# Connor-Guo/torcheval

Hardware: AMD Instinct MI355X
Metric: metric-updates/sec (whole node) MulticlassAccuracy bs=8192 at 1/2/4/8 MI355X (higher is better)
Workload: dtype fp32; 1 GPU; model=MulticlassAccuracy, global_batch=8192, num_classes=1000, batch_per_gpu=8192, average=micro, parallelism=dp1

## Files before the change

### csrc/bindings/counts.cpp

```cpp
#include <ATen/ATen.h>
#include <torch/csrc/utils/pybind.h>
#include <torch/library.h>

#include "tea_kernels.h"
#include "tea_torch.h"

namespace {

using namespace tea_torch;

void cls_counts(const Tensor& input, const Tensor& target, int64_t k, int64_t num_classes,
                const optional<Tensor>& micro_correct, const optional<Tensor>& micro_total,
                const optional<Tensor>& cls_correct, const optional<Tensor>& cls_label,
                const optional<Tensor>& cls_pred, const optional<Tensor>& confusion,
                const optional<Tensor>& err, int64_t max_blocks,
                const optional<Tensor>& micro_incorrect, const optional<Tensor>& micro_total2,
                const optional<Tensor>& cls_fp) {
  check_gpu(input, "input");
  check_gpu(target, "target");
  TORCH_CHECK(target.dim() == 1, "cls_counts: target must be 1-D");
  TORCH_CHECK(input.dim() == 1 || input.dim() == 2, "cls_counts: input must be 1-D or 2-D");
  TORCH_CHECK(input.size(0) == target.size(0), "cls_counts: first dims differ");
  TORCH_CHECK(target.is_contiguous(), "cls_counts: target must be contiguous");
  DeviceGuard guard(input.device());
  tea::ClsCountsArgs a;
  Tensor in = input;
  if (input.dim() == 2) {
    if (in.stride(1) != 1) in = in.contiguous();
    a.c = in.size(1);
    a.row_stride = in.stride(0);
    TORCH_CHECK(a.c < (int64_t(1) << 31), "cls_counts: too many classes");
    TORCH_CHECK(k >= 1 && k <= a.c || a.c == 0, "cls_counts: k out of range");
    if (num_classes <= 0) num_classes = a.c;
    TORCH_CHECK(num_classes == a.c, "cls_counts: num_classes must match input.size(1)");
  } else {
    if (!in.is_contiguous()) in = in.contiguous();
    TORCH_CHECK(k == 1, "cls_counts: k > 1 needs 2-D scores");
  }
  const int64_t C = num_classes;
  a.input = in.data_ptr();
  a.in_dt = dt_of(in);
  a.n = in.size(0);
  a.target = target.data_ptr();
  a.tg_dt = dt_of(target);
  a.k = static_cast<int>(k);
  a.num_classes = C;
  a.micro_correct = f32_out(micro_correct, input, 1, "micro_correct");
  a.micro_total = f32_out(micro_total, input, 1, "micro_total");
  a.cls_correct = f32_out(cls_correct, input, C, "cls_correct");
  a.cls_label = f32_out(cls_label, input, C, "cls_label");
  a.cls_pred = f32_out(cls_pred, input, C, "cls_pred");
  a.confusion = f32_out(confusion, input, C * C, "confusion");
  a.micro_incorrect = f32_out(micro_incorrect, input, 1, "micro_incorrect");
  a.micro_total2 = f32_out(micro_total2, input, 1, "micro_total2");
  a.cls_fp = f32_out(cls_fp, input, C, "cls_fp");
  TORCH_CHECK(!(k > 1 && (a.cls_pred || a.confusion || a.cls_fp)),
              "cls_counts: predictions are undefined for k > 1");
  TORCH_CHECK((a.cls_correct || a.cls_label || a.cls_pred || a.confusion || a.cls_fp) == false ||
                  C > 0,
              "cls_counts: num_classes required for histograms");
  if ((a.err = err_ptr(err, input, "cls_counts")) != nullptr) {
    if (err->numel() >= 3) a.err_max = a.err + 1;
    a.check_target = 1;
  }
  a.max_blocks = static_cast<int>(max_blocks);
  const hipStream_t stream = stream_for(input);
  if (a.micro_correct || a.micro_incorrect) a.fold_ws = fold_workspace(input, stream);
  const int rc = tea::launch_cls_counts(a, stream);
  TORCH_CHECK(rc != -1, "cls_counts: unsupported input dtype ", input.scalar_type());
  check_launch(rc, "cls_counts");
}

bool micro_accuracy_update(const Tensor& input, const Tensor& target, const Tensor& correct,
                           const Tensor& total, int64_t num_classes, const optional<Tensor>& pend) {
  if (!input.is_cuda() || input.dim() != 2 || target.dim() != 1) return false;
  const int64_t n = input.size(0), c = input.size(1);
  if (target.size(0) != n || c <= 0 || c >= (int64_t(1) << 31) || input.stride(1) != 1) return false;
  if (num_classes > 0 && c != num_classes) return false;
  const auto st = input.scalar_type();
  if (st != at::kFloat && st != at::kBFloat16 && st != at::kHalf) return false;
  switch (target.scalar_type()) {
    case at::kLong: case at::kInt: case at::kShort: case at::kChar: case at::kByte: case at::kBool:
      break;
    default: return false;
  }
  if (!target.is_contiguous()) return false;
  const auto dev = input.device();
  if (target.device() != dev || correct.device() != dev || total.device() != dev) return false;
  if (correct.scalar_type() != at::kFloat || total.scalar_type() != at::kFloat ||
      correct.numel() != 1 || total.numel() != 1)
    return false;
  DeviceGuard guard(dev);
  tea::ClsCountsArgs a;
  a.input = input.data_ptr();
  a.in_dt = dt_of(input);
  a.n = n;
  a.c = c;
  a.row_stride = input.stride(0);
  a.target = target.data_ptr();
  a.tg_dt = dt_of(target);
  a.k = 1;
  a.num_classes = c;
  a.micro_correct = correct.data_ptr<float>();
  a.micro_total = total.data_ptr<float>();
  const hipStream_t stream = stream_for(input);
  if (pend.has_value()) {
    if (pend->scalar_type() != at::kLong || pend->numel() < tea::kPendCells * tea::kPendStride ||
        pend->device() != dev || !pend->is_contiguous())
      return false;
    a.pend = reinterpret_cast<unsigned long long*>(pend->data_ptr<int64_t>());
  } else {
    a.fold_ws = fold_workspace(input, stream);
  }
  check_launch(tea::launch_cls_counts(a, stream), "micro_accuracy_update");
  return true;
}

void micro_accuracy_finish(const Tensor& pend, const Tensor& correct, const Tensor& total,
                           const optional<Tensor>& out) {
  check_gpu(pend, "pend");
  TORCH_CHECK(pend.scalar_type() == at::kLong && pend.is_contiguous() &&
                  pend.numel() >= tea::kPendCells * tea::kPendStride,
              "micro_accuracy_finish: pend must be int64 [>= 512]");
  TORCH_CHECK(correct.scalar_type() == at::kFloat && total.scalar_type() == at::kFloat && correct.numel() == 1 &&
                  total.numel() == 1 && correct.device() == pend.device() && total.device() == pend.device(),
              "micro_accuracy_finish: float32 scalar states on the pending cells' device");
  float* o = nullptr;
  if (out.has_value()) {
    TORCH_CHECK(out->scalar_type() == at::kFloat && out->numel() == 1 && out->device() == pend.device(),
                "micro_accuracy_finish: out must be a float32 scalar");
    o = out->data_ptr<float>();
  }
  DeviceGuard guard(pend.device());
  check_launch(tea::launch_micro_finish(reinterpret_cast<unsigned long long*>(pend.data_ptr<int64_t>()),
                                        correct.data_ptr<float>(), total.data_ptr<float>(), o, stream_for(pend)),
               "micro_accuracy_finish");
}

Tensor rank_scores(const Tensor& input, const Tensor& target, int64_t mode, int64_t k,
                   const optional<Tensor>& err) {
  check_gpu(input, "input");
  check_gpu(target, "target");
  TORCH_CHECK(input.dim() == 2 && target.dim() == 1 && input.size(0) == target.size(0),
              "rank_scores: input [n, c] and target [n] expected");
  TORCH_CHECK(mode == 0 || mode == 1, "rank_scores: mode must be 0 (hit) or 1 (reciprocal)");
  TORCH_CHECK(input.size(1) < (int64_t(1) << 31), "rank_scores: too many columns");
  DeviceGuard guard(input.device());
  Tensor in = input.stride(1) == 1 ? input : input.contiguous();
  Tensor tg = target.contiguous();
  tea::RankArgs a;
  a.input = in.data_ptr();
  a.in_dt = dt_of(in);
  a.n = in.size(0);
  a.c = in.size(1);
  a.row_stride = in.stride(0);
  a.target = tg.data_ptr();
  a.tg_dt = dt_of(tg);
  a.mode = static_cast<int>(mode);
  a.k = static_cast<int>(k);
  Tensor out = at::empty({a.n}, input.options().dtype(at::kFloat));
  a.out = out.data_ptr<float>();
  a.err = err_ptr(err, input, "rank_scores");
  const int rc = tea::launch_rank_scores(a, stream_for(input));
  TORCH_CHECK(rc != -1, "rank_scores: unsupported input dtype ", input.scalar_type());
  check_launch(rc, "rank_scores");
  return out;
}

void binary_counts(const Tensor& input, const Tensor& target, const optional<Tensor>& weight,
                   double threshold, const optional<Tensor>& tp, const optional<Tensor>& fp,
                   const optional<Tensor>& tn, const optional<Tensor>& fn,
                   const optional<Tensor>& total, int64_t strict, int64_t max_blocks,
                   const optional<Tensor>& tp2, const optional<Tensor>& fp2,
                   const optional<Tensor>& tn2, const optional<Tensor>& fn2) {
  check_gpu(input, "input");
  check_gpu(target, "target");
  TORCH_CHECK(input.numel() == target.numel(), "binary_counts: size mismatch");
  DeviceGuard guard(input.device());
  Tensor in = input.contiguous();
  Tensor tg = target.contiguous();
  Tensor w;
  tea::BinaryCountsArgs a;
  if (weight.has_value()) {
    w = weight->contiguous();
    TORCH_CHECK(w.numel() == in.numel(), "binary_counts: weight size mismatch");
    a.weight = w.data_ptr();
    a.w_dt = dt_of(w);
  }
  a.input = in.data_ptr();
  a.in_dt = dt_of(in);
  a.target = tg.data_ptr();
  a.tg_dt = dt_of(tg);
  a.n = in.numel();
  a.threshold = threshold_as(in, threshold);
  a.threshold64 = threshold;
  a.strict_binary = static_cast<int>(strict);
  a.out[0] = f32_out(tp, input, 1, "tp");
  a.out[1] = f32_out(fp, input, 1, "fp");
  a.out[2] = f32_out(tn, input, 1, "tn");
  a.out[3] = f32_out(fn, input, 1, "fn");
  a.total = f32_out(total, input, 1, "total");
  a.out2[0] = f32_out(tp2, input, 1, "tp2");
  a.out2[1] = f32_out(fp2, input, 1, "fp2");
  a.out2[2] = f32_out(tn2, input, 1, "tn2");
  a.out2[3] = f32_out(fn2, input, 1, "fn2");
  a.max_blocks = static_cast<int>(max_blocks);
  check_launch(tea::launch_binary_counts(a, stream_for(input)), "binary_counts");
}

void multilabel_counts(const Tensor& input, const Tensor& target, double threshold, int64_t k,
                       int64_t criteria, const Tensor& num_correct, const optional<Tensor>& num_total,
                       double total) {
  check_gpu(input, "input");
  check_gpu(target, "target");
  TORCH_CHECK(input.dim() == 2 && target.sizes() == input.sizes(),
              "multilabel_counts: input/target must be [n, c] of equal shape");
  TORCH_CHECK(input.stride(1) == 1 && target.stride(1) == 1,
              "multilabel_counts: rows must be contiguous");
  TORCH_CHECK(num_correct.scalar_type() == at::kFloat && num_correct.numel() == 1 &&
                  num_correct.device() == input.device(),
              "multilabel_counts: num_correct must be a float32 scalar on the input device");
  TORCH_CHECK(criteria >= 0 && criteria <= 4, "multilabel_counts: bad criteria");
  TORCH_CHECK(k == 0 || (k >= 1 && k <= input.size(1) && input.size(1) <= tea::multilabel_max_topk_cols()),
              "multilabel_counts: top-k needs 1 <= k <= c <= ", tea::multilabel_max_topk_cols());
  TORCH_CHECK(criteria != 1 || input.numel() < (int64_t{1} << 31),
              "multilabel_counts: hamming counts must fit 31 bits per launch");
  DeviceGuard guard(input.device());
  hipStream_t stream = stream_for(input);
  tea::MultilabelArgs a;
  a.x = input.data_ptr();
  a.x_dt = dt_of(input);
  a.x_row_stride = input.stride(0);
  a.t = target.data_ptr();
  a.t_dt = dt_of(target);
  a.t_row_stride = target.stride(0);
  a.n = input.size(0);
  a.c = input.size(1);
  a.threshold = threshold_as(input, threshold);
  a.k = static_cast<int>(k);
  a.criteria = static_cast<int>(criteria);
  a.num_correct = num_correct.data_ptr<float>();
  if (num_total.has_value()) {
    TORCH_CHECK(num_total->scalar_type() == at::kFloat && num_total->numel() == 1,
                "multilabel_counts: num_total must be a float32 scalar");
    a.num_total = num_total->data_ptr<float>();
    a.total = total;
  }
  a.fold_ws = fold_workspace(input, stream);
  const int rc = tea::launch_multilabel(a, stream);
  TORCH_CHECK(rc != -1, "multilabel_counts: unsupported dtypes ", input.scalar_type(), "/",
              target.scalar_type());
  check_launch(rc, "multilabel_counts");
}

void binned_counts(const Tensor& input, const Tensor& target, const Tensor& thr, int64_t mode,
                   const optional<Tensor>& tp, const optional<Tensor>& fp,
                   const optional<Tensor>& fn, int64_t uniform) {
  check_gpu(input, "input");
  TORCH_CHECK(input.dim() == 2, "binned_counts: input must be a 2-D view [n, c]");
  TORCH_CHECK(thr.dim() == 1 && thr.scalar_type() == at::kFloat && thr.is_contiguous(),
              "binned_counts: thresholds must be a contiguous float32 vector");
  DeviceGuard guard(input.device());
  tea::BinnedArgs a;
  a.input = input.data_ptr();
  a.in_dt = dt_of(input);
  a.n = input.size(0);
// ... 217 lines not shown
```

### csrc/include/tea_kernels.h

```cpp
#pragma once

#include <hip/hip_runtime_api.h>
#include <stdint.h>

#include "tea_types.h"

namespace tea {

struct ClsCountsArgs {
  const void* input = nullptr;
  DType in_dt = DType::f32;
  int64_t n = 0;
  int64_t c = 0;
  int64_t row_stride = 0;
  const void* target = nullptr;
  DType tg_dt = DType::i64;
  int k = 1;
  int64_t num_classes = 0;
  float* micro_correct = nullptr;
  float* micro_incorrect = nullptr;
  float* micro_total = nullptr;
  float* micro_total2 = nullptr;
  float* cls_correct = nullptr;
  float* cls_label = nullptr;
  float* cls_pred = nullptr;
  float* cls_fp = nullptr;
  float* confusion = nullptr;
  int* err = nullptr;
  int* err_max = nullptr;
  int check_target = 0;
  unsigned long long* fold_ws = nullptr;
  unsigned long long* pend = nullptr;
  int max_blocks = 0;
};
int launch_cls_counts(const ClsCountsArgs& a, hipStream_t stream);
constexpr int kPendCells = 64;
constexpr int kPendStride = 8;
int launch_micro_finish(unsigned long long* pend, float* correct, const float* total, float* out, hipStream_t stream);

struct BinaryCountsArgs {
  const void* input = nullptr;
  DType in_dt = DType::f32;
  const void* target = nullptr;
  DType tg_dt = DType::f32;
  const void* weight = nullptr;
  DType w_dt = DType::f32;
  int64_t n = 0;
  float threshold = 0.5f;
  double threshold64 = 0.5;
  int strict_binary = 0;
  float* out[4] = {nullptr, nullptr, nullptr, nullptr};
  float* out2[4] = {nullptr, nullptr, nullptr, nullptr};
  float* total = nullptr;
  int max_blocks = 0;
};
int launch_binary_counts(const BinaryCountsArgs& a, hipStream_t stream);

struct RankArgs {
  const void* input = nullptr;
  DType in_dt = DType::f32;
  int64_t n = 0;
  int64_t c = 0;
  int64_t row_stride = 0;
  const void* target = nullptr;
  DType tg_dt = DType::i64;
  int mode = 0;
  int k = 0;
  float* out = nullptr;
  int* err = nullptr;
};
int launch_rank_scores(const RankArgs& a, hipStream_t stream);

}

namespace tea {

struct AucScanArgs {
  int payload_kind = 0;
  const void* sorted = nullptr;
  DType key_dt = DType::f32;
  int64_t key_stride = 0;
  const int64_t* order = nullptr;
  const int32_t* order32 = nullptr;
  int64_t order_stride = 0;
  const void* target = nullptr;
  DType tg_dt = DType::f32;
  int64_t target_stride = 0;
  const void* weight = nullptr;
  DType w_dt = DType::f32;
  int64_t weight_stride = 0;
  int class_mode = 0;
  int64_t rows = 0;
  int64_t n = 0;
  double* out_auroc = nullptr;
  double* out_auprc = nullptr;
  const uint32_t* sort_fault = nullptr;
  const double* init = nullptr;
  double* out_raw = nullptr;
  void* ab = nullptr;
  void* tsum = nullptr;
  void* tstart = nullptr;
  void* tarea = nullptr;
  void* totals = nullptr;
  int32_t* tcnt = nullptr;
  int32_t* cstart = nullptr;
  int64_t* sizes = nullptr;
  const int64_t* row_off = nullptr;
  float* out_prec = nullptr;
  float* out_rec = nullptr;
  void* out_thr = nullptr;
  float min_precision = 0.f;
  float* s_rec = nullptr;
  void* s_thr = nullptr;
  int32_t* gstar = nullptr;
  int32_t* glo = nullptr;
  float* out_max_recall = nullptr;
  void* out_best_thr = nullptr;
};
int64_t auc_scan_workspace_bytes(int64_t rows, int64_t n);
int launch_auc_scan(AucScanArgs a, void* workspace, hipStream_t stream);
int64_t curve_workspace_bytes(int64_t rows, int64_t n, bool rafp);
constexpr int kMergeTile = 2048;
int64_t merge_splits_count(int64_t n);
int launch_merge_desc(const float* ka, const uint32_t* va, int64_t na, uint32_t base_a, const float* kb,
                      const uint32_t* vb, int64_t nb, uint32_t base_b, float* ko, uint32_t* vo, int64_t* splits,
                      hipStream_t stream);
int launch_curve_count(AucScanArgs& a, void* workspace, bool rafp, hipStream_t stream);
int launch_curve_emit(AucScanArgs a, void* workspace, bool rafp, hipStream_t stream);
int launch_rafp(AucScanArgs a, void* workspace, hipStream_t stream);

}

namespace tea {

struct BinnedArgs {
  const void* input = nullptr;
  DType in_dt = DType::f32;
  int64_t n = 0;
  int64_t c = 0;
  int64_t in_row_stride = 0;
  int64_t in_col_stride = 0;
  const void* target = nullptr;
  DType tg_dt = DType::i64;
  int mode = 0;
  int64_t tg_row_stride = 0;
  int64_t tg_col_stride = 0;
  const float* thr = nullptr;
  int T = 0;
  int uniform = 0;
  unsigned* ws = nullptr;
  unsigned* slab = nullptr;
  float* tp = nullptr;
  float* fp = nullptr;
  float* fn = nullptr;
  int64_t out_k_stride = 0;
  int64_t out_c_stride = 0;
};
int64_t binned_workspace_words(int T, int64_t c);
int64_t binned_slab_words(int T, int64_t c);
struct BinnedFinalizeArgs {
  const float* tp = nullptr;
  const float* fp = nullptr;
  const float* fn = nullptr;
  int64_t k_stride = 0, r_stride = 0;
  int T = 0;
  int64_t rows = 0;
  double* out_auroc = nullptr;
  float* out_auprc = nullptr;
  float* out_prec = nullptr;
  float* out_rec = nullptr;
};
int launch_binned_finalize(const BinnedFinalizeArgs& a, hipStream_t stream);
int launch_binned(const BinnedArgs& a, hipStream_t stream);

}

namespace tea {

struct MomentsArgs {
  const void* x = nullptr;
  DType x_dt = DType::f32;
  int64_t x_row_stride = 0, x_col_stride = 0;
  const void* t = nullptr;
  DType t_dt = DType::f32;
  int64_t t_row_stride = 0, t_col_stride = 0;
  const void* w = nullptr;
  DType w_dt = DType::f32;
  int64_t w_stride = 0;
// ... 715 lines not shown
```

### csrc/kernels/classification.hip

```cpp
#include <algorithm>
#include <cstdlib>

#include "tea_common.h"
#include "tea_fold.h"
#include "tea_kernels.h"
#include "tea_rowload.h"

namespace tea {

namespace {

constexpr int kBlock = 256;
constexpr int kWavesPerBlock = kBlock / kWave;
constexpr int kChunkLoads = 4;
constexpr int kNarrowMaxC = 32;

template <int KIND, int VEC>
__device__ __forceinline__ void load_vec(const void* row, int col, float (&v)[VEC]) {
  if constexpr (KIND == 0 && VEC == 4) {
    const float4 x = *reinterpret_cast<const float4*>(static_cast<const float*>(row) + col);
    v[0] = x.x;
    v[1] = x.y;
    v[2] = x.z;
    v[3] = x.w;
// ... 271 lines not shown
        if (base + CHUNK < C) load_chunk<KIND, VEC, UNAL>(rp, base + CHUNK, C, lane, nx);
        finish_chunk<VEC, UNAL>(v, base, C, lane);
#pragma unroll
        for (int u = 0; u < kChunkLoads; ++u)
#pragma unroll
          for (int e = 0; e < VEC; ++e) cnt += v[u][e] > xt;
      }
      cnt = wave_sum(cnt);
      correct = t_ok && cnt < a.k;
    }
    if (lane == 0) {
      correct_acc += correct;
      rows_acc += 1;
      row_hist(h, a.num_classes, t, pred, correct, a.err, a.check_target, a.err_max);
    }
  }
  block_micro(a, correct_acc, rows_acc);
}


template <int CTRL>
__device__ __forceinline__ float dpp_f32(float x) {
  return __int_as_float(__builtin_amdgcn_update_dpp(0, __float_as_int(x), CTRL, 0xf, 0xf, false));
}

__device__ __forceinline__ float wave_max_dpp(float x) {
  x = fmaximum(x, dpp_f32<0xB1>(x));
  x = fmaximum(x, dpp_f32<0x4E>(x));
  x = fmaximum(x, dpp_f32<0x141>(x));
  x = fmaximum(x, dpp_f32<0x140>(x));
  const float r0 = __int_as_float(__builtin_amdgcn_readlane(__float_as_int(x), 0));
  const float r1 = __int_as_float(__builtin_amdgcn_readlane(__float_as_int(x), 16));
  const float r2 = __int_as_float(__builtin_amdgcn_readlane(__float_as_int(x), 32));
  const float r3 = __int_as_float(__builtin_amdgcn_readlane(__float_as_int(x), 48));
  return fmaximum(fmaximum(r0, r1), fmaximum(r2, r3));
}

template <int NV>
struct RowVals;
template <>
struct RowVals<16> {
  typedef float type __attribute__((ext_vector_type(16)));
};
template <>
struct RowVals<32> {
  typedef float type __attribute__((ext_vector_type(32)));
};

template <int KIND, typename TGT, bool UNAL = false>
__device__ __forceinline__ void micro_rows(const void* __restrict__ input, const TGT* __restrict__ target, int64_t n,
                                           int C, int64_t row_stride, uint32_t& correct_acc, uint32_t& rows_acc) {
  constexpr int VEC = KIND == 0 ? 4 : 8;
  constexpr int NV = kChunkLoads * VEC;
  constexpr int STEP = kWave * VEC;
  typedef typename RowVals<NV>::type vec_t;
  const int lane = lane_id();
  const int64_t nwaves = static_cast<int64_t>(gridDim.x) * kWavesPerBlock;
  for (int64_t row = static_cast<int64_t>(blockIdx.x) * kWavesPerBlock + wave_id(); row < n; row += nwaves) {
    const char* rp = static_cast<const char*>(input) + row * row_stride * kind_bytes<KIND>;
    float f[kChunkLoads][VEC];
#pragma unroll
    for (int u = 0; u < kChunkLoads; ++u) load_row_vec<KIND, VEC, UNAL>(rp, u * STEP + lane * VEC, C, f[u]);
    const int64_t t = target[row];
    if constexpr (UNAL) unal_fix_tail<kChunkLoads>(f, 0, C, lane);
    vec_t v;
#pragma unroll
    for (int u = 0; u < kChunkLoads; ++u)
#pragma unroll
      for (int e = 0; e < VEC; ++e) v[u * VEC + e] = f[u][e];
    float m = fmaximum(v[0], v[1]);
#pragma unroll
    for (int e = 2; e < NV; ++e) m = fmaximum(m, v[e]);
    const float wm = wave_max_dpp(m);
    bool correct = false;
    if (__builtin_expect(wm != wm, 0)) {
      correct = row_argmax_exact<KIND>(rp, C, lane) == t;
    } else if (t >= 0 && t < C) {
      const int tu = static_cast<int>(t);
      const float sel = v[(tu / STEP) * VEC + (tu % VEC)];
      const float xt = __int_as_float(__builtin_amdgcn_readlane(__float_as_int(sel), (tu % STEP) / VEC));
      if (xt == wm) {
        int cnt = 0;
#pragma unroll
        for (int u = 0; u < kChunkLoads; ++u) {
          const int valid = min(max((C - u * STEP + VEC - 1) / VEC, 0), kWave);
          const uint64_t lanes = valid >= kWave ? ~0ull : ((1ull << valid) - 1);
#pragma unroll
          for (int e = 0; e < VEC; ++e) cnt += __builtin_popcountll(__ballot(v[u * VEC + e] == wm) & lanes);
        }
        correct = cnt == 1 || row_argmax_exact<KIND>(rp, C, lane) == t;
      }
    }
    if (lane == 0) {
      correct_acc += correct;
      rows_acc += 1;
    }
  }
}

template <int KIND, typename TGT, bool UNAL>
__global__ __launch_bounds__(kBlock) void cls_micro_kernel(ClsCountsArgs a) {
  uint32_t correct_acc = 0, rows_acc = 0;
  micro_rows<KIND, TGT, UNAL>(a.input, static_cast<const TGT*>(a.target), a.n, static_cast<int>(a.c), a.row_stride,
                        correct_acc, rows_acc);
  block_micro(a, correct_acc, rows_acc);
}

template <int KIND, typename TGT, bool UNAL>
__device__ __forceinline__ bool micro_row(int C, const char* __restrict__ rp, int64_t t, int lane) {
  constexpr int VEC = KIND == 0 ? 4 : 8;
  constexpr int NV = kChunkLoads * VEC;
  constexpr int STEP = kWave * VEC;
  typedef typename RowVals<NV>::type vec_t;
  float f[kChunkLoads][VEC];
#pragma unroll
  for (int u = 0; u < kChunkLoads; ++u) load_row_vec<KIND, VEC, UNAL>(rp, u * STEP + lane * VEC, C, f[u]);
  if constexpr (UNAL) unal_fix_tail<kChunkLoads>(f, 0, C, lane);
  vec_t v;
#pragma unroll
  for (int u = 0; u < kChunkLoads; ++u)
#pragma unroll
    for (int e = 0; e < VEC; ++e) v[u * VEC + e] = f[u][e];
  float m = fmaximum(v[0], v[1]);
#pragma unroll
  for (int e = 2; e < NV; ++e) m = fmaximum(m, v[e]);
  if (__builtin_expect(__ballot(m != m) != 0, 0)) return row_argmax_exact<KIND>(rp, C, lane) == t;
  if (!(t >= 0 && t < C)) return false;
  const int tu = static_cast<int>(t);
  const float sel = v[(tu / STEP) * VEC + (tu % VEC)];
  const float xt = __int_as_float(__builtin_amdgcn_readlane(__float_as_int(sel), (tu % STEP) / VEC));
  if (__ballot(m > xt) != 0) return false;
  bool tie = false;
#pragma unroll
  for (int u = 0; u < kChunkLoads; ++u)
#pragma unroll
    for (int e = 0; e < VEC; ++e) tie |= (v[u * VEC + e] == xt) & (u * STEP + lane * VEC + e < tu);
  return __ballot(tie) == 0;
}

template <int KIND, typename TGT, int WPB, bool UNAL>
__global__ __launch_bounds__(WPB * kWave) void cls_micro_pend_kernel(const char* __restrict__ input,
                                                                     const TGT* __restrict__ target,
                                                                     unsigned long long* __restrict__ pend,
                                                                     float* __restrict__ total, int64_t n,
                                                                     int64_t row_stride, int32_t c,
                                                                     int32_t nwaves ) {
  const int lane = lane_id();
  const int64_t row0 = static_cast<int64_t>(blockIdx.x) * WPB + wave_id();
  const int64_t r0 = row0 < n ? row0 : n - 1;
  const bool c0 = micro_row<KIND, TGT, UNAL>(c, input + r0 * row_stride * kind_bytes<KIND>, target[r0], lane);
  uint32_t correct_acc = (row0 < n && c0) ? 1u : 0u;
  for (int64_t row = row0 + nwaves; row < n; row += nwaves)
    correct_acc += micro_row<KIND, TGT, UNAL>(c, input + row * row_stride * kind_bytes<KIND>, target[row], lane);
  if (lane == 0 && correct_acc)
    atomicAdd(pend + ((blockIdx.x * WPB + wave_id()) % kPendCells) * kPendStride,
              static_cast<unsigned long long>(correct_acc));
  if (blockIdx.x == 0 && threadIdx.x == 0 && total) atomicAdd(total, static_cast<float>(n));
}

__global__ __launch_bounds__(kWave) void micro_finish_kernel(unsigned long long* pend, float* correct,
                                                             const float* total, float* out) {
  unsigned long long* cell = pend + threadIdx.x * kPendStride;
  const unsigned long long s = wave_sum(*cell);
  *cell = 0ull;
  if (threadIdx.x == 0) {
    const float c = correct[0] + static_cast<float>(s);
    correct[0] = c;
    if (out) out[0] = c / total[0];
  }
}

template <int KIND, int VEC, bool TOPK, bool PRED = true, bool UNAL = false>
__global__ __launch_bounds__(kBlock) void cls_wide_kernel(ClsCountsArgs a) {
  cls_wide_body<KIND, VEC, TOPK, PRED, UNAL>(a);
}

template <int KIND, bool TOPK>
__global__ __launch_bounds__(kBlock) void cls_narrow_kernel(ClsCountsArgs a) {
  __shared__ float s_correct[kNarrowMaxC], s_label[kNarrowMaxC], s_pred[kNarrowMaxC];
  __shared__ float s_fp[kNarrowMaxC];
  __shared__ float s_conf[kNarrowMaxC * kNarrowMaxC];
  const int C = static_cast<int>(a.c);
  for (int i = threadIdx.x; i < C * C; i += kBlock) s_conf[i] = 0.f;
  if (threadIdx.x < kNarrowMaxC) {
    s_correct[threadIdx.x] = 0.f;
    s_label[threadIdx.x] = 0.f;
    s_pred[threadIdx.x] = 0.f;
    s_fp[threadIdx.x] = 0.f;
  }
  __syncthreads();
  const Hist lh{a.cls_correct ? s_correct : nullptr, a.cls_label ? s_label : nullptr,
                a.cls_pred ? s_pred : nullptr, a.cls_fp ? s_fp : nullptr,
                a.confusion ? s_conf : nullptr};
  uint32_t correct_acc = 0, rows_acc = 0;
  const int64_t stride = static_cast<int64_t>(gridDim.x) * kBlock;
  for (int64_t row = static_cast<int64_t>(blockIdx.x) * kBlock + threadIdx.x; row < a.n;
       row += stride) {
    const void* rp = static_cast<const char*>(a.input) + row * a.row_stride * kind_bytes<KIND>;
    const int64_t t = load_target(a.target, a.tg_dt, row);
    bool correct;
    int64_t pred = -1;
    if constexpr (!TOPK) {
      float bv = -__builtin_huge_valf();
      int bi = 0x7fffffff;
      for (int c = 0; c < C; ++c) {
        const float v = load1<KIND>(rp, c);
        if (argmax_better(v, c, bv, bi)) {
          bv = v;
          bi = c;
        }
      }
      pred = bi;
      correct = pred == t;
    } else {
      const bool t_ok = t >= 0 && t < C;
      const float xt = t_ok ? load1<KIND>(rp, t) : __builtin_nanf("");
      int cnt = 0;
      for (int c = 0; c < C; ++c) cnt += load1<KIND>(rp, c) > xt;
      correct = t_ok && cnt < a.k;
    }
    correct_acc += correct;
    rows_acc += 1;
    row_hist(lh, C, t, pred, correct, a.err, a.check_target, a.err_max);
  }
  __syncthreads();
  for (int i = threadIdx.x; i < C; i += kBlock) {
    if (a.cls_correct && s_correct[i] != 0.f) atomicAdd(a.cls_correct + i, s_correct[i]);
    if (a.cls_label && s_label[i] != 0.f) atomicAdd(a.cls_label + i, s_label[i]);
    if (a.cls_pred && s_pred[i] != 0.f) atomicAdd(a.cls_pred + i, s_pred[i]);
    if (a.cls_fp && s_fp[i] != 0.f) atomicAdd(a.cls_fp + i, s_fp[i]);
  }
  if (a.confusion)
    for (int i = threadIdx.x; i < C * C; i += kBlock)
      if (s_conf[i] != 0.f) atomicAdd(a.confusion + i, s_conf[i]);
  block_micro(a, correct_acc, rows_acc);
}

__global__ __launch_bounds__(kBlock) void cls_labels_kernel(ClsCountsArgs a) {
  const Hist h{a.cls_correct, a.cls_label, a.cls_pred, a.cls_fp, a.confusion};
  uint32_t correct_acc = 0, rows_acc = 0;
  const int64_t stride = static_cast<int64_t>(gridDim.x) * kBlock;
  for (int64_t i = static_cast<int64_t>(blockIdx.x) * kBlock + threadIdx.x; i < a.n; i += stride) {
    const int64_t p = load_as_i64(a.input, a.in_dt, i);
    const int64_t t = load_target(a.target, a.tg_dt, i);
    const bool correct = p == t;
    correct_acc += correct;
    rows_acc += 1;
    row_hist(h, a.num_classes, t, p, correct, a.err, a.check_target, a.err_max);
  }
  block_micro(a, correct_acc, rows_acc);
}

template <bool F64>
__global__ __launch_bounds__(kBlock) void binary_counts_kernel(BinaryCountsArgs a) {
  float acc[4] = {0.f, 0.f, 0.f, 0.f};
  const int64_t stride = static_cast<int64_t>(gridDim.x) * kBlock;
  for (int64_t i = static_cast<int64_t>(blockIdx.x) * kBlock + threadIdx.x; i < a.n; i += stride) {
    const double t = load_as_f64(a.target, a.tg_dt, i);
    const float w = a.weight ? load_as_f32(a.weight, a.w_dt, i) : 1.f;
    bool pos;
    if constexpr (F64) pos = !(load_as_f64(a.input, DType::f64, i) < a.threshold64);
    else pos = !(load_as_f32(a.input, a.in_dt, i) < a.threshold);
    const bool t1 = t == 1.0, t0 = t == 0.0;
    const float other = a.strict_binary ? 0.f : w;
    if (pos) {
      acc[0] += t1 ? w : 0.f;
      acc[1] += t0 ? w : (t1 ? 0.f : other);
    } else {
      acc[2] += t0 ? w : 0.f;
      acc[3] += t1 ? w : (t0 ? 0.f : other);
    }
  }
  __shared__ float lds[4][kWavesPerBlock];
#pragma unroll
  for (int j = 0; j < 4; ++j) {
    const float s = wave_sum(acc[j]);
    if (lane_id() == 0) lds[j][threadIdx.x >> 6] = s;
  }
  __syncthreads();
  if (threadIdx.x < 4) {
    float s = 0.f;
#pragma unroll
    for (int w = 0; w < kWavesPerBlock; ++w) s += lds[threadIdx.x][w];
    float* dst = a.out[threadIdx.x];
    if (dst && s != 0.f) atomicAdd(dst, s);
    float* dst2 = a.out2[threadIdx.x];
    if (dst2 && s != 0.f) atomicAdd(dst2, s);
  }
  if (threadIdx.x == 0 && blockIdx.x == 0 && a.total) atomicAdd(a.total, static_cast<float>(a.n));
}

template <int KIND, int VEC, bool UNAL = false>
void launch_wide(const ClsCountsArgs& a, int grid, hipStream_t s) {
  constexpr int kChunkCols = kWave * VEC * kChunkLoads;
  const bool pred_free = a.cls_pred == nullptr && a.cls_fp == nullptr && a.confusion == nullptr &&
                         a.c <= kChunkCols;
  static const bool micro_on = [] {
    const char* e = std::getenv("TORCHEVAL_AMD_K1_MICRO");
    return e == nullptr || std::atoi(e) != 0;
  }();
  const bool micro_only = micro_on && pred_free && VEC > 1 && a.k == 1 && a.cls_correct == nullptr &&
                          a.cls_label == nullptr && a.err == nullptr && a.err_max == nullptr && !a.check_target;
  if (micro_only && a.pend && (a.tg_dt == DType::i64 || a.tg_dt == DType::i32)) {
    const char* in = static_cast<const char*>(a.input);
    const int32_t c = static_cast<int32_t>(a.c);
    static const int wpb = [] {
      const char* e = std::getenv("TORCHEVAL_AMD_K1_WPB");
      return (e && std::atoi(e) == 4) ? 4 : 8;
    }();
    if (wpb == 8) {
      const int g8 = stream_grid(a.n, 8, a.max_blocks > 0 ? (a.max_blocks + 1) / 2 : 1024);
      if (a.tg_dt == DType::i64)
        hipLaunchKernelGGL((cls_micro_pend_kernel<KIND, int64_t, 8, UNAL>), dim3(g8), dim3(8 * kWave), 0, s, in,
                           static_cast<const int64_t*>(a.target), a.pend, a.micro_total, a.n, a.row_stride, c, g8 * 8);
      else
        hipLaunchKernelGGL((cls_micro_pend_kernel<KIND, int32_t, 8, UNAL>), dim3(g8), dim3(8 * kWave), 0, s, in,
                           static_cast<const int32_t*>(a.target), a.pend, a.micro_total, a.n, a.row_stride, c, g8 * 8);
      return;
    }
    if (a.tg_dt == DType::i64)
      hipLaunchKernelGGL((cls_micro_pend_kernel<KIND, int64_t, kWavesPerBlock, UNAL>), dim3(grid), dim3(kBlock), 0, s, in,
                         static_cast<const int64_t*>(a.target), a.pend, a.micro_total, a.n, a.row_stride, c,
                         grid * kWavesPerBlock);
    else
      hipLaunchKernelGGL((cls_micro_pend_kernel<KIND, int32_t, kWavesPerBlock, UNAL>), dim3(grid), dim3(kBlock), 0, s, in,
                         static_cast<const int32_t*>(a.target), a.pend, a.micro_total, a.n, a.row_stride, c,
                         grid * kWavesPerBlock);
    return;
  }
  if (micro_only && a.tg_dt == DType::i64) {
    hipLaunchKernelGGL((cls_micro_kernel<KIND, int64_t, UNAL>), dim3(grid), dim3(kBlock), 0, s, a);
    return;
  }
  if (micro_only && a.tg_dt == DType::i32) {
    hipLaunchKernelGGL((cls_micro_kernel<KIND, int32_t, UNAL>), dim3(grid), dim3(kBlock), 0, s, a);
    return;
  }
  if (a.k > 1)
    hipLaunchKernelGGL((cls_wide_kernel<KIND, VEC, true, true, UNAL>), dim3(grid), dim3(kBlock), 0, s, a);
  else if (pred_free)
    hipLaunchKernelGGL((cls_wide_kernel<KIND, VEC, false, false, UNAL>), dim3(grid), dim3(kBlock), 0, s, a);
  else
    hipLaunchKernelGGL((cls_wide_kernel<KIND, VEC, false, true, UNAL>), dim3(grid), dim3(kBlock), 0, s, a);
}

template <int KIND>
void launch_narrow(const ClsCountsArgs& a, int grid, hipStream_t s) {
  if (a.k > 1)
    hipLaunchKernelGGL((cls_narrow_kernel<KIND, true>), dim3(grid), dim3(kBlock), 0, s, a);
  else
    hipLaunchKernelGGL((cls_narrow_kernel<KIND, false>), dim3(grid), dim3(kBlock), 0, s, a);
}

}

int launch_cls_counts(const ClsCountsArgs& a, hipStream_t stream) {
  if (a.n <= 0) return 0;
  if (a.c > 0) {
    const uintptr_t base = reinterpret_cast<uintptr_t>(a.input);
    const int kind = a.in_dt == DType::f32 ? 0 : a.in_dt == DType::bf16 ? 1 : a.in_dt == DType::f16 ? 2 : -1;
    if (kind < 0) return -1;
    if (a.c <= kNarrowMaxC) {
      const int cap = a.max_blocks > 0 ? a.max_blocks : 512;
      const int grid = stream_grid(a.n, kBlock, cap);
      if (kind == 0) launch_narrow<0>(a, grid, stream);
      else if (kind == 1) launch_narrow<1>(a, grid, stream);
      else launch_narrow<2>(a, grid, stream);
    } else {
      const int cap = a.max_blocks > 0 ? a.max_blocks : 2048;
      const int grid = stream_grid(a.n, kWavesPerBlock, cap);
      const int vw = kind == 0 ? 4 : 8;
      const bool vec = (a.c % vw == 0) && (a.row_stride % vw == 0) && (base % 16 == 0);
      if (kind == 0) vec ? launch_wide<0, 4>(a, grid, stream) : launch_wide<0, 4, true>(a, grid, stream);
      else if (kind == 1) vec ? launch_wide<1, 8>(a, grid, stream) : launch_wide<1, 1>(a, grid, stream);
      else vec ? launch_wide<2, 8>(a, grid, stream) : launch_wide<2, 1>(a, grid, stream);
    }
  } else {
    const int cap = a.max_blocks > 0 ? a.max_blocks : 1024;
    const int grid = stream_grid(a.n, kBlock, cap);
    hipLaunchKernelGGL(cls_labels_kernel, dim3(grid), dim3(kBlock), 0, stream, a);
  }
  return static_cast<int>(hipGetLastError());
}

int launch_micro_finish(unsigned long long* pend, float* correct, const float* total, float* out,
                        hipStream_t stream) {
  hipLaunchKernelGGL(micro_finish_kernel, dim3(1), dim3(kPendCells), 0, stream, pend, correct, total, out);
  return static_cast<int>(hipGetLastError());
}

int launch_binary_counts(const BinaryCountsArgs& a, hipStream_t stream) {
  if (a.n <= 0) return 0;
  const int cap = a.max_blocks > 0 ? a.max_blocks : 256;
  const int grid = stream_grid(a.n, kBlock * 4, cap);
  if (a.in_dt == DType::f64) hipLaunchKernelGGL(binary_counts_kernel<true>, dim3(grid), dim3(kBlock), 0, stream, a);
  else hipLaunchKernelGGL(binary_counts_kernel<false>, dim3(grid), dim3(kBlock), 0, stream, a);
  return static_cast<int>(hipGetLastError());
}

}
```

Baseline: 171,400 updates/s.

## Add software-pipelined wave-per-row micro accuracy kernel for wide class counts

Adds a dedicated micro-accuracy kernel for rows wider than one chunk (for example C=1000 fp32). Each wave walks one row, keeps two or three register chunk buffers so the next loads are in flight while the current chunk is compared, and stops early once the row is known to be wrong. Counts go into the pending int64 cells instead of the generic wide kernel with its fold workspace. The fold workspace allocation is now skipped when this path is taken. This adds register pressure and an early-exit branch, and the default depth of 3 can be changed through an environment variable.

New measurement: 172,000 updates/s, median of 6. Within noise of the previous version (+0.4%).

```diff
diff --git a/csrc/bindings/counts.cpp b/csrc/bindings/counts.cpp
--- a/csrc/bindings/counts.cpp
+++ b/csrc/bindings/counts.cpp
@@ -109,9 +109,8 @@
         pend->device() != dev || !pend->is_contiguous())
       return false;
     a.pend = reinterpret_cast<unsigned long long*>(pend->data_ptr<int64_t>());
-  } else {
-    a.fold_ws = fold_workspace(input, stream);
-  }
+  }
+  if (!tea::cls_counts_uses_pend(a)) a.fold_ws = fold_workspace(input, stream);
   check_launch(tea::launch_cls_counts(a, stream), "micro_accuracy_update");
   return true;
 }
diff --git a/csrc/include/tea_kernels.h b/csrc/include/tea_kernels.h
--- a/csrc/include/tea_kernels.h
+++ b/csrc/include/tea_kernels.h
@@ -34,6 +34,7 @@
   int max_blocks = 0;
 };
 int launch_cls_counts(const ClsCountsArgs& a, hipStream_t stream);
+bool cls_counts_uses_pend(const ClsCountsArgs& a);
 constexpr int kPendCells = 64;
 constexpr int kPendStride = 8;
 int launch_micro_finish(unsigned long long* pend, float* correct, const float* total, float* out, hipStream_t stream);
diff --git a/csrc/kernels/classification.hip b/csrc/kernels/classification.hip
--- a/csrc/kernels/classification.hip
+++ b/csrc/kernels/classification.hip
@@ -447,6 +447,120 @@
   uint32_t correct_acc = (row0 < n && c0) ? 1u : 0u;
   for (int64_t row = row0 + nwaves; row < n; row += nwaves)
     correct_acc += micro_row<KIND, TGT, UNAL>(c, input + row * row_stride * kind_bytes<KIND>, target[row], lane);
+  if (lane == 0 && correct_acc)
+    atomicAdd(pend + ((blockIdx.x * WPB + wave_id()) % kPendCells) * kPendStride,
+              static_cast<unsigned long long>(correct_acc));
+  if (blockIdx.x == 0 && threadIdx.x == 0 && total) atomicAdd(total, static_cast<float>(n));
+}
+
+template <int KIND, bool UNAL>
+__device__ __forceinline__ void load_chunk_raw(const char* __restrict__ rp, int base, int C, int lane,
+                                               uint4 (&b)[kChunkLoads]) {
+  constexpr int VEC = KIND == 0 ? 4 : 8;
+  constexpr int STEP = kWave * VEC;
+#pragma unroll
+  for (int u = 0; u < kChunkLoads; ++u) {
+    const int col = base + u * STEP + lane * VEC;
+    if constexpr (UNAL) {
+      const int lc = col + 4 <= C ? col : (col < C ? C - 4 : 0);
+      const float4 q = load_f4u(reinterpret_cast<const float*>(rp) + lc);
+      b[u] = make_uint4(__float_as_uint(q.x), __float_as_uint(q.y), __float_as_uint(q.z), __float_as_uint(q.w));
+    } else {
+      b[u] = *reinterpret_cast<const uint4*>(rp + static_cast<int64_t>(col < C ? col : 0) * kind_bytes<KIND>);
+    }
+  }
+  __builtin_amdgcn_sched_barrier(0);
+}
+
+template <int KIND, int VEC>
+__device__ __forceinline__ void expand_raw(const uint4& x, float (&v)[VEC]) {
+  if constexpr (KIND == 0) {
+    v[0] = __uint_as_float(x.x);
+    v[1] = __uint_as_float(x.y);
+    v[2] = __uint_as_float(x.z);
+    v[3] = __uint_as_float(x.w);
+  } else {
+    unpack8<KIND>(x, v);
+  }
+}
+
+template <int KIND, bool UNAL>
+__device__ __forceinline__ void micro_wide_chunk(const uint4 (&b)[kChunkLoads], int base, int C, int lane, float xt,
+                                                 int tu, bool& lost) {
+  constexpr int VEC = KIND == 0 ? 4 : 8;
+  constexpr int STEP = kWave * VEC;
+  float v[kChunkLoads][VEC];
+#pragma unroll
+  for (int u = 0; u < kChunkLoads; ++u) expand_raw<KIND, VEC>(b[u], v[u]);
+  float mc = fmaximum(v[0][0], v[0][1]);
+#pragma unroll
+  for (int u = 0; u < kChunkLoads; ++u)
+#pragma unroll
+    for (int e = (u == 0 ? 2 : 0); e < VEC; ++e) mc = fmaximum(mc, v[u][e]);
+  if (__ballot(!(mc < xt)) != 0) {
+    if constexpr (UNAL) unal_fix_tail<kChunkLoads>(v, base, C, lane);
+    bool hl = false;
+    if (xt != xt) {
+#pragma unroll
+      for (int u = 0; u < kChunkLoads; ++u)
+#pragma unroll
+        for (int e = 0; e < VEC; ++e) hl |= (v[u][e] != v[u][e]) & (base + u * STEP + lane * VEC + e < tu);
+    } else {
+#pragma unroll
+      for (int u = 0; u < kChunkLoads; ++u)
+#pragma unroll
+        for (int e = 0; e < VEC; ++e)
+          hl |= !(v[u][e] <= xt) | ((v[u][e] == xt) & (base + u * STEP + lane * VEC + e < tu));
+    }
+    lost |= __ballot(hl) != 0;
+  }
+}
+
+template <int KIND, typename TGT, bool UNAL, int DEPTH>
+__global__ __launch_bounds__(8 * kWave) void cls_micro_wide_pend_kernel(const char* __restrict__ input,
+                                                                        const TGT* __restrict__ target,
+                                                                        unsigned long long* __restrict__ pend,
+                                                                        float* __restrict__ total, int64_t n,
+                                                                        int64_t row_stride, int32_t c,
+                                                                        int32_t nwaves ) {
+  static_assert(DEPTH == 2 || DEPTH == 3, "two or three chunk buffers");
+  constexpr int WPB = 8;
+  constexpr int VEC = KIND == 0 ? 4 : 8;
+  constexpr int CHUNK = kWave * VEC * kChunkLoads;
+  const int lane = lane_id();
+  uint32_t correct_acc = 0;
+  for (int64_t row = static_cast<int64_t>(blockIdx.x) * WPB + wave_id(); row < n; row += nwaves) {
+    const char* rp = input + row * row_stride * kind_bytes<KIND>;
+    uint4 b0[kChunkLoads], b1[kChunkLoads], b2[kChunkLoads];
+    load_chunk_raw<KIND, UNAL>(rp, 0, c, lane, b0);
+    if constexpr (DEPTH == 3) load_chunk_raw<KIND, UNAL>(rp, CHUNK, c, lane, b1);
+    const int64_t t = target[row];
+    const bool t_ok = t >= 0 && t < c;
+    const int tu = t_ok ? static_cast<int>(t) : 0;
+    const float xt = __int_as_float(__builtin_amdgcn_readfirstlane(__float_as_int(load1<KIND>(rp, tu))));
+    if (!t_ok) continue;
+    bool lost = false;
+    if constexpr (DEPTH == 3) {
+      for (int base = 0;; base += 3 * CHUNK) {
+        load_chunk_raw<KIND, UNAL>(rp, base + 2 * CHUNK, c, lane, b2);
+        micro_wide_chunk<KIND, UNAL>(b0, base, c, lane, xt, tu, lost);
+        load_chunk_raw<KIND, UNAL>(rp, base + 3 * CHUNK, c, lane, b0);
+        micro_wide_chunk<KIND, UNAL>(b1, base + CHUNK, c, lane, xt, tu, lost);
+        load_chunk_raw<KIND, UNAL>(rp, base + 4 * CHUNK, c, lane, b1);
+        micro_wide_chunk<KIND, UNAL>(b2, base + 2 * CHUNK, c, lane, xt, tu, lost);
+        if (lost || base + 3 * CHUNK >= c) break;
+      }
+    } else {
+      for (int base = 0;; base += 2 * CHUNK) {
+        load_chunk_raw<KIND, UNAL>(rp, base + CHUNK, c, lane, b1);
+        micro_wide_chunk<KIND, UNAL>(b0, base, c, lane, xt, tu, lost);
+        load_chunk_raw<KIND, UNAL>(rp, base + 2 * CHUNK, c, lane, b0);
+        micro_wide_chunk<KIND, UNAL>(b1, base + CHUNK, c, lane, xt, tu, lost);
+        if (lost || base + 2 * CHUNK >= c) break;
+      }
+    }
+    correct_acc += !lost;
+  }
   if (lane == 0 && correct_acc)
     atomicAdd(pend + ((blockIdx.x * WPB + wave_id()) % kPendCells) * kPendStride,
               static_cast<unsigned long long>(correct_acc));
@@ -585,17 +699,52 @@
   if (threadIdx.x == 0 && blockIdx.x == 0 && a.total) atomicAdd(a.total, static_cast<float>(a.n));
 }
 
+bool micro_counts_only(const ClsCountsArgs& a) {
+  static const bool micro_on = [] {
+    const char* e = std::getenv("TORCHEVAL_AMD_K1_MICRO");
+    return e == nullptr || std::atoi(e) != 0;
+  }();
+  return micro_on && a.cls_pred == nullptr && a.cls_fp == nullptr && a.confusion == nullptr && a.k == 1 &&
+         a.cls_correct == nullptr && a.cls_label == nullptr && a.err == nullptr && a.err_max == nullptr &&
+         !a.check_target;
+}
+
+bool micro_to_pend(const ClsCountsArgs& a) {
+  return a.pend != nullptr && (a.tg_dt == DType::i64 || a.tg_dt == DType::i32) && a.c < (int64_t(1) << 30) &&
+         micro_counts_only(a);
+}
+
+template <int KIND, typename TGT, bool UNAL>
+void launch_micro_wide(const ClsCountsArgs& a, hipStream_t s) {
+  static const int depth = [] {
+    const char* e = std::getenv("TORCHEVAL_AMD_K1_WIDE_DEPTH");
+    return (e && std::atoi(e) == 2) ? 2 : 3;
+  }();
+  const int g8 = stream_grid(a.n, 8, a.max_blocks > 0 ? (a.max_blocks + 1) / 2 : 1024);
+  const char* in = static_cast<const char*>(a.input);
+  const TGT* tg = static_cast<const TGT*>(a.target);
+  const int32_t c = static_cast<int32_t>(a.c);
+  if (depth == 3)
+    hipLaunchKernelGGL((cls_micro_wide_pend_kernel<KIND, TGT, UNAL, 3>), dim3(g8), dim3(8 * kWave), 0, s, in, tg, a.pend,
+                       a.micro_total, a.n, a.row_stride, c, g8 * 8);
+  else
+    hipLaunchKernelGGL((cls_micro_wide_pend_kernel<KIND, TGT, UNAL, 2>), dim3(g8), dim3(8 * kWave), 0, s, in, tg, a.pend,
+                       a.micro_total, a.n, a.row_stride, c, g8 * 8);
+}
+
 template <int KIND, int VEC, bool UNAL = false>
 void launch_wide(const ClsCountsArgs& a, int grid, hipStream_t s) {
   constexpr int kChunkCols = kWave * VEC * kChunkLoads;
   const bool pred_free = a.cls_pred == nullptr && a.cls_fp == nullptr && a.confusion == nullptr &&
                          a.c <= kChunkCols;
-  static const bool micro_on = [] {
-    const char* e = std::getenv("TORCHEVAL_AMD_K1_MICRO");
-    return e == nullptr || std::atoi(e) != 0;
-  }();
-  const bool micro_only = micro_on && pred_free && VEC > 1 && a.k == 1 && a.cls_correct == nullptr &&
-                          a.cls_label == nullptr && a.err == nullptr && a.err_max == nullptr && !a.check_target;
+  const bool micro_only = pred_free && VEC > 1 && micro_counts_only(a);
+  if constexpr (VEC > 1) {
+    if (a.c > kChunkCols && micro_to_pend(a)) {
+      if (a.tg_dt == DType::i64) launch_micro_wide<KIND, int64_t, UNAL>(a, s);
+      else launch_micro_wide<KIND, int32_t, UNAL>(a, s);
+      return;
+    }
+  }
   if (micro_only && a.pend && (a.tg_dt == DType::i64 || a.tg_dt == DType::i32)) {
     const char* in = static_cast<const char*>(a.input);
     const int32_t c = static_cast<int32_t>(a.c);
@@ -649,10 +798,20 @@
 
 }
 
+static bool rows_take_16b_loads(const ClsCountsArgs& a) {
+  const int vw = a.in_dt == DType::f32 ? 4 : 8;
+  return (a.c % vw == 0) && (a.row_stride % vw == 0) && (reinterpret_cast<uintptr_t>(a.input) % 16 == 0);
+}
+
+bool cls_counts_uses_pend(const ClsCountsArgs& a) {
+  if (a.c <= kNarrowMaxC || !micro_to_pend(a)) return false;
+  if (a.in_dt == DType::f32) return true;
+  return (a.in_dt == DType::bf16 || a.in_dt == DType::f16) && rows_take_16b_loads(a);
+}
+
 int launch_cls_counts(const ClsCountsArgs& a, hipStream_t stream) {
   if (a.n <= 0) return 0;
   if (a.c > 0) {
-    const uintptr_t base = reinterpret_cast<uintptr_t>(a.input);
     const int kind = a.in_dt == DType::f32 ? 0 : a.in_dt == DType::bf16 ? 1 : a.in_dt == DType::f16 ? 2 : -1;
     if (kind < 0) return -1;
     if (a.c <= kNarrowMaxC) {
@@ -664,8 +823,7 @@
     } else {
       const int cap = a.max_blocks > 0 ? a.max_blocks : 2048;
       const int grid = stream_grid(a.n, kWavesPerBlock, cap);
-      const int vw = kind == 0 ? 4 : 8;
-      const bool vec = (a.c % vw == 0) && (a.row_stride % vw == 0) && (base % 16 == 0);
+      const bool vec = rows_take_16b_loads(a);
       if (kind == 0) vec ? launch_wide<0, 4>(a, grid, stream) : launch_wide<0, 4, true>(a, grid, stream);
       else if (kind == 1) vec ? launch_wide<1, 8>(a, grid, stream) : launch_wide<1, 1>(a, grid, stream);
       else vec ? launch_wide<2, 8>(a, grid, stream) : launch_wide<2, 1>(a, grid, stream);
```
